# gstoica27/ReLUQP-py

Hardware: AMD Instinct MI355X
Metric: QP solves/sec (batch=4096 random dense QPs n=100 m=300) (higher is better)
Workload: dtype f32; 1 GPU; batch=4096/GPU random dense QPs n=100 m=300 (n_eq=25), feasible rand_qp seeds 0.., eps_abs=0.001, cold start, reference defaults; 4 distinct batches in rotation, every solve without dispatch history (= first solve of a fresh handle); global_batch=4096, parallelism=batch-split x1, no collectives, kernel=resident2, tile=same, low_memory=False, fresh_batches=4, dispatch_history=False, rho_window=5

## Files before the change

### reluqp-py_amd/csrc/rqp_resident2.hip

```cpp
#include <cstdio>
#include <cstdlib>
#include <type_traits>
#include <vector>

#include "rqp_common.h"

typedef float f2 __attribute__((ext_vector_type(2)));
typedef _Float16 h2 __attribute__((ext_vector_type(2)));

__device__ __forceinline__ float fma_mix_lo(h2 k, float v, float acc) {
    asm("v_fma_mix_f32 %0, %1, %2, %0 op_sel_hi:[1,0,0]" : "+v"(acc) : "v"(k), "v"(v));
    return acc;
}
__device__ __forceinline__ float fma_mix_hi(h2 k, float v, float acc) {
    asm("v_fma_mix_f32 %0, %1, %2, %0 op_sel:[1,0,0] op_sel_hi:[1,0,0]" : "+v"(acc) : "v"(k), "v"(v));
    return acc;
}
template <int CTRL>
__device__ __forceinline__ float dpp2(float v) {
    return __builtin_bit_cast(float, __builtin_amdgcn_update_dpp(0, __builtin_bit_cast(int, v), CTRL, 0xF, 0xF, true));
}
__device__ __forceinline__ float swsum32(float a, float b) {
    asm volatile("s_nop 1\n\tv_permlane32_swap_b32 %0, %1" : "+v"(a), "+v"(b));
    return a + b;
}
__device__ __forceinline__ float swsum16(float a, float b) {
    asm volatile("s_nop 1\n\tv_permlane16_swap_b32 %0, %1" : "+v"(a), "+v"(b));
    return a + b;
}
__device__ __forceinline__ float swmax32(float a, float b) {
    asm volatile("s_nop 1\n\tv_permlane32_swap_b32 %0, %1" : "+v"(a), "+v"(b));
    return fmaxf(a, b);
}
__device__ __forceinline__ float swmax16(float a, float b) {
    asm volatile("s_nop 1\n\tv_permlane16_swap_b32 %0, %1" : "+v"(a), "+v"(b));
    return fmaxf(a, b);
}
__device__ __forceinline__ float wave_max(float v) {
    v = fmaxf(v, dpp2<0xB1>(v));
    v = fmaxf(v, dpp2<0x4E>(v));
    v = fmaxf(v, dpp2<0x141>(v));
    v = fmaxf(v, dpp2<0x128>(v));
    float a = v, b = v;
    asm volatile("s_nop 1\n\tv_permlane16_swap_b32 %0, %1" : "+v"(a), "+v"(b));
    v = fmaxf(a, b);
    a = v; b = v;
    asm volatile("s_nop 1\n\tv_permlane32_swap_b32 %0, %1" : "+v"(a), "+v"(b));
    return fmaxf(a, b);
}
__device__ __forceinline__ unsigned wave_or(unsigned v) {
    v |= (unsigned)__builtin_amdgcn_update_dpp(0, (int)v, 0xB1, 0xF, 0xF, true);
    v |= (unsigned)__builtin_amdgcn_update_dpp(0, (int)v, 0x4E, 0xF, 0xF, true);
    v |= (unsigned)__builtin_amdgcn_update_dpp(0, (int)v, 0x141, 0xF, 0xF, true);
    v |= (unsigned)__builtin_amdgcn_update_dpp(0, (int)v, 0x128, 0xF, 0xF, true);
    unsigned a = v, b = v;
    asm volatile("s_nop 1\n\tv_permlane16_swap_b32 %0, %1" : "+v"(a), "+v"(b));
    v = a | b;
    a = v; b = v;
    asm volatile("s_nop 1\n\tv_permlane32_swap_b32 %0, %1" : "+v"(a), "+v"(b));
    return a | b;
}
template <typename T>
__device__ __forceinline__ T tmax2(T a, T b) {
    return (a != a) ? a : ((b != b) ? b : (a > b ? a : b));
}

template <int RB_, int CQ_, int KR_, int KC_>
struct Res2Cfg {
    static constexpr int RB = RB_, CQ = CQ_, KR = KR_, KC = KC_;
    static constexpr int NT = 256, NW = 4, NQ = 2, PL = 32;
    static constexpr int RP = RB / 2, KP = KR / 2;
    static constexpr int CW = NQ * CQ;
    static constexpr int N = NW * CW;
    static constexpr int M = PL * RB;
    static constexpr int SW = 8 * KR + 4;
    static constexpr int ND = NW * SW;
    static constexpr int AE2 = RP * CQ;
    static constexpr int KE2 = KP * KC;
    static constexpr int HR = 4, HP = HR / 2;
    static constexpr int HE2 = HP * CQ;
    static constexpr int HU = HE2 / 2;
    static constexpr int H1 = (CQ + 1) / 2, H2 = (H1 + 1) / 2;
    static constexpr int MATREGS = 2 * (RP * CQ + KP * KC);
    static constexpr int WAVES_PER_SIMD = (MATREGS > 100) ? 2 : ((MATREGS > 30) ? 3 : 4);
    static_assert(RB % 2 == 0 && KR % 2 == 0 && HP == 2 && HU == CQ && PL * HR >= N, "row pairs");
    static_assert(8 * KR >= CW && 8 * KC >= N && M <= 2 * NT && KC == CQ && NQ == 2, "tile shape");
    static constexpr size_t lds_bytes() {
        return (size_t)M * 8 * 4 + ND * 8 + 16 * 8
               + (size_t)M * 4 * 5
               + (size_t)ND * 4 * 6
               + (size_t)NW * M * 4 + 96 * 4
               + (size_t)HU * NT * 16;
    }
};

constexpr int NSEG = 25;
template <class C, bool DIAG, bool KH, bool KD = false>
__global__ void __launch_bounds__(256, C::WAVES_PER_SIMD) k_admm_res2(SolveArgs a, const float* __restrict__ Apack,
                                                      const float* __restrict__ Kpack,
                                                      const float* __restrict__ Hpack, unsigned long long* dbg,
                                                      const float* __restrict__ Kscale) {
    constexpr int RB = C::RB, CQ = C::CQ, KR = C::KR, KC = C::KC, NT = C::NT, NW = C::NW, RP = C::RP, KP = C::KP;
    constexpr int CW = C::CW, M = C::M, ND = C::ND, SW = C::SW, AE2 = C::AE2, KE2 = C::KE2, HU = C::HU, HP = C::HP, HR = C::HR, H1 = C::H1, H2 = C::H2;
    extern __shared__ __attribute__((aligned(16))) unsigned char smem_raw[];
    double* zt64 = (double*)smem_raw;
    double* lam64 = zt64 + M;
    double* z64 = lam64 + M;
    double* inv64 = z64 + M;
    double* x64 = inv64 + M;
    double* redd = x64 + ND;
    float* lT = (float*)(redd + 16);
    float* uT = lT + M;
    float* rv32 = uT + M;
    float* nu = rv32 + M;
    float* cT = nu + M;
    float* xin = cT + M;
    float* xnat = xin + ND;
    float* dxv = xnat + ND;
    float* hx = dxv + ND;
    float* gT = hx + ND;
    float* dvec = gT + ND;
    float* part = dvec + ND;
    float* red = part + NW * M;
    float* Hs = red + 96;
    static_assert(((size_t)M * 8 * 4 + ND * 8 + 16 * 8 + (size_t)M * 4 * 5 + ND * 4 * 6 + NW * M * 4 + 96 * 4) % 16 == 0,
                  "H image must start 16-byte aligned");

    const int n = a.n, m = a.m;
    const int b = a.order ? a.order[blockIdx.x] : (int)blockIdx.x, tid = threadIdx.x;
    const int wave = tid >> 6, lane = tid & 63;
    const int q = lane & 1, pl = lane >> 1, rr = lane >> 3, cc = lane & 7;
    const size_t mat = (a.sA == 0) ? 0 : (size_t)b;
    const float* cg = (const float*)a.c + (size_t)b * m;
    int k0 = 0;
    bool exact = false;
    if (a.cont == 1) {
        if (a.info.status[b] != RQP_STATUS_CONTINUE) {
            if (!(a.warm_starting || a.keep_state)) {
                for (int i = tid; i < n; i += NT) a.x[(size_t)b * n + i] = 0.0;
                for (int i = tid; i < m; i += NT) {
                    a.z[(size_t)b * m + i] = 0.0;
                    a.lam[(size_t)b * m + i] = 0.0;
                }
                if (tid == 0) a.rho_ind[b] = a.rho_ind0;
            }
            return;
        }
        k0 = a.cont_iter[b];
    } else if (a.cont == 2) {
        if (a.gate && *a.gate == 0) return;
        if (a.cstat[b] == 0) return;
        const int ci = a.cont_iter[b];
        if (ci >= 0) {
            k0 = ci;
            exact = true;
        }
    }
    const int wb = a.wbase ? a.wbase[mat] : 0;
    if (a.cstat && a.mode == 0) {
        const int sl = a.rho_ind[b] - wb;
        if (sl < 0 || sl >= a.kwin) {
            if (tid == 0) {
                a.cstat[b] = 1;
                if (!exact) a.cont_iter[b] = -1;
                atomicAdd(a.ncont, 1);
            }
            return;
        }
    }

    f2 ar[RP][CQ];
    {
        const f2* Ap = (const f2*)(Apack + mat * (size_t)AE2 * NT * 2) + tid;
#pragma unroll
        for (int rp = 0; rp < RP; ++rp)
#pragma unroll
            for (int c = 0; c < CQ; ++c) ar[rp][c] = Ap[(size_t)(rp * CQ + c) * NT];
        const float4* Hp = (const float4*)(Hpack + mat * (size_t)HU * NT * 4);
#pragma unroll
        for (int u = 0; u < HU; ++u) ((float4*)Hs)[u * NT + tid] = Hp[u * NT + tid];
    }
    int ri = a.rho_ind[b];
    float* rhoL = red + 64;
    if (tid < 32) rhoL[tid] = (tid < a.nrho) ? (float)a.rhos[tid] : 0.f;
    typedef typename std::conditional<KH, h2, f2>::type kpair_t;
    kpair_t kr[KP][KC];
    float kscale = 1.f;
    auto load_K = [&](int jl) {
        int j = jl - wb;
        j = j < 0 ? 0 : (j >= a.kwin ? a.kwin - 1 : j);
        if constexpr (!KD) {
            int tid_k = tid;
            asm volatile("" : "+v"(tid_k));
            const kpair_t* Kp = (const kpair_t*)Kpack + (mat * a.kwin + j) * (size_t)KE2 * NT + tid_k;
#pragma unroll
            for (int kp = 0; kp < KP; ++kp)
#pragma unroll
                for (int c = 0; c < KC; ++c) kr[kp][c] = Kp[(size_t)(kp * KC + c) * NT];
            if constexpr (KH) kscale = Kscale[mat * a.kwin + j];
        } else {
            int lane_o = lane, wave_o = wave;
            asm volatile("" : "+v"(lane_o), "+v"(wave_o));
            const int rr = lane_o >> 3, cc = lane_o & 7, wave = wave_o;
            const float* Kj = (const float*)a.K + ((a.sK == 0) ? (size_t)0 : (size_t)b * a.sK) + (size_t)j * n * a.ldn;
            typedef float f4u __attribute__((ext_vector_type(4), aligned(4)));
#pragma unroll
            for (int kp = 0; kp < KP; ++kp) {
                const int lr = KR * rr + 2 * kp, r = CW * wave + lr;
                const bool ok0 = lr < CW && r < n, ok1 = lr + 1 < CW && r + 1 < n;
                const float* row0 = Kj + (size_t)(r < n ? r : n - 1) * a.ldn + KC * cc;
                const float* row1 = Kj + (size_t)(r + 1 < n ? r + 1 : n - 1) * a.ldn + KC * cc;
                float t0[KC], t1[KC];
#pragma unroll
                for (int c = 0; c + 4 <= KC; c += 4) {
                    const f4u u0 = *(const f4u*)(row0 + c), u1 = *(const f4u*)(row1 + c);
#pragma unroll
                    for (int e = 0; e < 4; ++e) { t0[c + e] = u0[e]; t1[c + e] = u1[e]; }
                }
#pragma unroll
                for (int c = KC - KC % 4; c < KC; ++c) { t0[c] = row0[c]; t1[c] = row1[c]; }
                const f2 msk = {ok0 ? 1.f : 0.f, ok1 ? 1.f : 0.f};
#pragma unroll
                for (int c = 0; c < KC; ++c) kr[kp][c] = (f2){t0[c], t1[c]} * msk;
            }
        }
    };
    load_K(ri);

    auto set_rho_rows = [&](int j) {
        const float rho = (float)a.rhos[j];
        for (int i = tid; i < M; i += NT) {
            const float rv = rho * ((i < m) ? cg[i] : 1.f);
            rv32[i] = rv;
            inv64[i] = 1.0 / (double)rv;
        }
    };
    for (int i = tid; i < M; i += NT) {
        const bool in = i < m;
        zt64[i] = (exact && in) ? a.ax[(size_t)b * m + i] : 0.0;
        z64[i] = in ? a.z[(size_t)b * m + i] : 0.0;
        lam64[i] = in ? a.lam[(size_t)b * m + i] : 0.0;
        lT[i] = in ? ((const float*)a.l)[(size_t)b * m + i] : 0.f;
        uT[i] = in ? ((const float*)a.u)[(size_t)b * m + i] : 0.f;
        nu[i] = 0.f;
        cT[i] = in ? cg[i] : 1.f;
    }
    set_rho_rows(ri);
    for (int i = tid; i < ND; i += NT) {
        const int col = CW * (i / SW) + (i % SW);
        const bool in = (i % SW) < CW && col < n;
        const double xv = in ? a.x[(size_t)b * n + col] : 0.0;
        x64[i] = xv;
        xin[i] = (float)xv;
        xnat[i] = (i < n) ? (float)a.x[(size_t)b * n + i] : 0.f;
        gT[i] = in ? ((const float*)a.g)[(size_t)b * n + col] : 0.f;
        hx[i] = 0.f;
        dxv[i] = 0.f;
        dvec[i] = 0.f;
    }

    int colw, ncolw;
    {
        const int b5 = (lane >> 5) & 1, b4 = (lane >> 4) & 1;
        const int cbase = H2 * b4 + H1 * b5;
        int nval = b4 ? (H1 - H2) : H2;
        if (b5 && cbase + nval > CQ) nval = CQ - cbase;
        ncolw = ((lane & 0xE) == 0) ? nval : 0;
        colw = SW * wave + CQ * q + cbase;
    }
    __syncthreads();

    auto load_vc = [&](const float* v, float (&vc)[CQ]) __attribute__((always_inline)) {
#pragma unroll
        for (int c = 0; c < CQ; ++c) vc[c] = v[SW * wave + CQ * q + c];
    };
    auto prod_A = [&](const float (&vc)[CQ]) __attribute__((always_inline)) {
        f2 acc[RP];
#pragma unroll
        for (int rp = 0; rp < RP; ++rp) {
            f2 s = {0.f, 0.f};
#pragma unroll
            for (int c = 0; c < CQ; ++c) s = __builtin_elementwise_fma(ar[rp][c], (f2){vc[c], vc[c]}, s);
            s.x += dpp2<0xB1>(s.x);
            s.y += dpp2<0xB1>(s.y);
            acc[rp] = s;
        }
        if (q == 0) {
            f2* dst = (f2*)(part + wave * M + RB * pl);
#pragma unroll
            for (int rp = 0; rp < RP; ++rp) dst[rp] = acc[rp];
        }
    };
    auto prod_At = [&](auto use_a, auto use_h, const float* w, float* out, bool addg) {
        constexpr bool USE_A = decltype(use_a)::value, USE_H = decltype(use_h)::value;
        f2 wr[RP];
        f2 wx[HP];
        if constexpr (USE_A) {
#pragma unroll
            for (int rp = 0; rp < RP; ++rp) wr[rp] = ((const f2*)(w + RB * pl))[rp];
        }
        if constexpr (USE_H) {
            const float4 xv = *(const float4*)(xnat + HR * pl);
            wx[0] = (f2){xv.x, xv.y};
            wx[1] = (f2){xv.z, xv.w};
        }
        auto hload = [&](int c) -> float4 { return ((const float4*)Hs)[c * NT + tid]; };
        auto colsum = [&](int c, const float4& hv) -> float {
            f2 t2 = {0.f, 0.f};
            if constexpr (USE_A) {
#pragma unroll
                for (int rp = 0; rp < RP; ++rp) t2 = __builtin_elementwise_fma(ar[rp][c], wr[rp], t2);
            }
            if constexpr (USE_H) {
                t2 = __builtin_elementwise_fma((f2){hv.x, hv.y}, wx[0], t2);
                t2 = __builtin_elementwise_fma((f2){hv.z, hv.w}, wx[1], t2);
            }
            return t2.x + t2.y;
        };
        float s1[H1];
        auto colsum2 = [&](int c0, int c1, const float4& h0, const float4& h1, float& a0, float& a1) __attribute__((always_inline)) {
            f2 t0 = {0.f, 0.f}, t1 = {0.f, 0.f};
            if constexpr (USE_A) {
#pragma unroll
                for (int rp = 0; rp < RP; ++rp) {
                    t0 = __builtin_elementwise_fma(ar[rp][c0], wr[rp], t0);
                    t1 = __builtin_elementwise_fma(ar[rp][c1], wr[rp], t1);
                }
            }
            if constexpr (USE_H) {
                t0 = __builtin_elementwise_fma((f2){h0.x, h0.y}, wx[0], t0);
                t1 = __builtin_elementwise_fma((f2){h1.x, h1.y}, wx[0], t1);
                t0 = __builtin_elementwise_fma((f2){h0.z, h0.w}, wx[1], t0);
                t1 = __builtin_elementwise_fma((f2){h1.z, h1.w}, wx[1], t1);
            }
            a0 = t0.x + t0.y;
            a1 = t1.x + t1.y;
        };
        float4 hcur = {0.f, 0.f, 0.f, 0.f}, hnext = {0.f, 0.f, 0.f, 0.f};
        if constexpr (USE_H) {
            hcur = hload(0);
            if (H1 < CQ) hnext = hload(H1);
        }
#pragma unroll
        for (int i = 0; i < H1; ++i) {
            const bool pair = (i + H1 < CQ);
            if (pair) {
                float4 hc2 = hcur, hn2 = hnext;
                if constexpr (USE_H) {
                    if (i + 1 < H1) hc2 = hload(i + 1);
                    if (i + 1 + H1 < CQ) hn2 = hload(i + 1 + H1);
                }
                float a0, a1;
                colsum2(i, i + H1, hcur, hnext, a0, a1);
                s1[i] = swsum32(a0, a1);
                hcur = hc2;
                hnext = hn2;
            } else {
                const float a0 = colsum(i, hcur);
                s1[i] = swsum32(a0, a0);
            }
        }
        float gpre[H2];
#pragma unroll
        for (int i = 0; i < H2; ++i) gpre[i] = addg ? gT[colw + i] : 0.f;
        float s2[H2];
#pragma unroll
        for (int i = 0; i < H2; ++i) s2[i] = (i + H2 < H1) ? swsum16(s1[i], s1[i + H2]) : swsum16(s1[i], s1[i]);
#pragma unroll
        for (int i = 0; i < H2; ++i) {
            float v = s2[i];
            v += dpp2<0x4E>(v);
            v += dpp2<0x124>(v);
            v += dpp2<0x128>(v);
            s2[i] = v;
        }
        if (ncolw > 0) {
#pragma unroll
            for (int i = 0; i < H2; ++i)
                if (i < ncolw) out[colw + i] = s2[i] + gpre[i];
        }
    };
    constexpr std::true_type YES{};
    auto prod_At_chk = [&](const float* w, float* outA, float* outH) {
        f2 wr[RP];
        f2 wx[HP];
#pragma unroll
        for (int rp = 0; rp < RP; ++rp) wr[rp] = ((const f2*)(w + RB * pl))[rp];
        {
            const float4 xv = *(const float4*)(xnat + HR * pl);
            wx[0] = (f2){xv.x, xv.y};
            wx[1] = (f2){xv.z, xv.w};
        }
        auto hload = [&](int c) -> float4 { return ((const float4*)Hs)[c * NT + tid]; };
        float sA[H1], sH[H1];
        float4 hcur = hload(0), hnext = {0.f, 0.f, 0.f, 0.f};
        if (H1 < CQ) hnext = hload(H1);
#pragma unroll
        for (int i = 0; i < H1; ++i) {
            const bool pair = (i + H1 < CQ);
            float4 hc2 = hcur, hn2 = hnext;
            if (i + 1 < H1) hc2 = hload(i + 1);
            if (i + 1 + H1 < CQ) hn2 = hload(i + 1 + H1);
            f2 a0 = {0.f, 0.f}, a1 = {0.f, 0.f};
            f2 h0 = __builtin_elementwise_fma((f2){hcur.x, hcur.y}, wx[0], (f2){0.f, 0.f}), h1 = {0.f, 0.f};
            if (pair) h1 = __builtin_elementwise_fma((f2){hnext.x, hnext.y}, wx[0], h1);
#pragma unroll
            for (int rp = 0; rp < RP; ++rp) {
                a0 = __builtin_elementwise_fma(ar[rp][i], wr[rp], a0);
                if (pair) a1 = __builtin_elementwise_fma(ar[rp][i + H1], wr[rp], a1);
            }
            h0 = __builtin_elementwise_fma((f2){hcur.z, hcur.w}, wx[1], h0);
            if (pair) h1 = __builtin_elementwise_fma((f2){hnext.z, hnext.w}, wx[1], h1);
            const float ca0 = a0.x + a0.y, ch0 = h0.x + h0.y;
            sA[i] = pair ? swsum32(ca0, a1.x + a1.y) : swsum32(ca0, ca0);
            sH[i] = pair ? swsum32(ch0, h1.x + h1.y) : swsum32(ch0, ch0);
            hcur = hc2;
            hnext = hn2;
        }
        float tA[H2], tH[H2];
#pragma unroll
        for (int i = 0; i < H2; ++i) {
            tA[i] = (i + H2 < H1) ? swsum16(sA[i], sA[i + H2]) : swsum16(sA[i], sA[i]);
            tH[i] = (i + H2 < H1) ? swsum16(sH[i], sH[i + H2]) : swsum16(sH[i], sH[i]);
        }
#pragma unroll
        for (int i = 0; i < H2; ++i) {
            float va = tA[i], vh = tH[i];
            va += dpp2<0x4E>(va);
            vh += dpp2<0x4E>(vh);
            va += dpp2<0x124>(va);
            vh += dpp2<0x124>(vh);
            va += dpp2<0x128>(va);
            vh += dpp2<0x128>(vh);
            tA[i] = va;
            tH[i] = vh;
        }
        if (ncolw > 0) {
#pragma unroll
            for (int i = 0; i < H2; ++i)
                if (i < ncolw) {
                    outA[colw + i] = tA[i] + 0.f;
                    outH[colw + i] = tH[i] + 0.f;
                }
        }
    };
    auto prod_K = [&](const float* v, float (&s)[KR]) {
        float vc[KC];
#pragma unroll
        for (int c = 0; c < KC; ++c) vc[c] = v[SW * (cc >> 1) + CQ * (cc & 1) + c];
#pragma unroll
        for (int kp = 0; kp < KP; ++kp) {
            f2 t = {0.f, 0.f};
            if constexpr (KH) {
#pragma unroll
                for (int c = 0; c < KC; ++c) {
                    t.x = fma_mix_lo(kr[kp][c], vc[c], t.x);
                    t.y = fma_mix_hi(kr[kp][c], vc[c], t.y);
                }
                t.x *= kscale;
                t.y *= kscale;
            } else {
#pragma unroll
                for (int c = 0; c < KC; ++c) t = __builtin_elementwise_fma(kr[kp][c], (f2){vc[c], vc[c]}, t);
            }
            s[2 * kp] = t.x;
            s[2 * kp + 1] = t.y;
        }
#pragma unroll
        for (int r = 0; r < KR; ++r) s[r] += dpp2<0xB1>(s[r]);
#pragma unroll
        for (int r = 0; r < KR; ++r) s[r] += dpp2<0x4E>(s[r]);
#pragma unroll
        for (int r = 0; r < KR; ++r) s[r] += dpp2<0x141>(s[r]);
    };
    float cv[3] = {0.f, 0.f, 0.f};
    auto row_body = [&](auto nr, bool init, bool do_a, bool do_b, bool chk) __attribute__((always_inline)) {
        constexpr int R = decltype(nr)::value;
        double zt[R], z[R], lmv[R], iv[R];
        float adx[R][NW], lo[R], hi[R], rvf[R];
#pragma unroll
        for (int q = 0; q < R; ++q) {
            const int i = tid + q * NT;
            zt[q] = zt64[i];
            lmv[q] = lam64[i];
            if (do_a) {
                iv[q] = inv64[i];
                lo[q] = lT[i];
                hi[q] = uT[i];
            } else {
                z[q] = z64[i];
            }
            rvf[q] = rv32[i];
            if (init || do_a) {
#pragma unroll
                for (int w = 0; w < NW; ++w) adx[q][w] = part[w * M + i];
            }
        }
        asm volatile("s_waitcnt lgkmcnt(0)" ::: "memory");
#pragma unroll
        for (int q = 0; q < R; ++q) {
            asm volatile("" : "+v"(zt[q]), "+v"(lmv[q]), "+v"(rvf[q]));
            if (do_a) asm volatile("" : "+v"(iv[q]), "+v"(lo[q]), "+v"(hi[q]));
            else asm volatile("" : "+v"(z[q]));
            if (init || do_a) asm volatile("" : "+v"(adx[q][0]), "+v"(adx[q][1]), "+v"(adx[q][2]), "+v"(adx[q][3]));
        }
#pragma unroll
        for (int q = 0; q < R; ++q) {
            const int i = tid + q * NT;
            if (init || do_a) {
                const float ad = ((adx[q][0] + adx[q][1]) + adx[q][2]) + adx[q][3];
                zt[q] = (init ? 0.0 : zt[q]) + (double)ad;
                zt64[i] = zt[q];
            }
            if (do_a) {
                const double v = zt[q] + lmv[q] * iv[q];
                z[q] = v;
                if (v < (double)lo[q]) z[q] = (double)lo[q];
                if (v > (double)hi[q]) z[q] = (double)hi[q];
                z64[i] = z[q];
            }
            if (do_b) {
                const double rv = (double)rvf[q];
                const double pr = zt[q] - z[q];
                const double lh = lmv[q] + rv * pr;
                lam64[i] = lh;
                nu[i] = (float)(lh + rv * pr);
            }
        }
        if (chk) {
            int tid_w = tid;
            asm volatile("" : "+v"(tid_w));
#pragma unroll
            for (int q = 0; q < R; ++q) {
                const int i = tid_w + q * NT;
                const float we = (a.scE && i < m) ? (float)(1.0 / a.scE[mat * m + i]) : 1.f;
                nu[i] = (float)lmv[q];
                cv[0] = tmax2(cv[0], fabsf((float)(zt[q] - z[q])) * we);
                cv[1] = tmax2(cv[1], fabsf((float)zt[q]) * we);
                cv[2] = tmax2(cv[2], fabsf((float)z[q]) * we);
            }
        }
    };
    auto row_pass = [&](bool init, bool do_a, bool do_b, bool chk = false) __attribute__((always_inline)) {
        if constexpr (M > NT) {
            static_assert(M <= 2 * NT, "at most two rows per lane");
            if (tid + NT < M) {
                row_body(std::integral_constant<int, 2>{}, init, do_a, do_b, chk);
                return;
            }
        }
        if (tid < M) row_body(std::integral_constant<int, 1>{}, init, do_a, do_b, chk);
    };

    __builtin_amdgcn_s_waitcnt(0x0F70);
    unsigned long long t_last = 0, t_acc[NSEG] = {};
    bool k_pend = false;
    bool diag_on = true;
    auto stamp = [&](int seg) {
        if constexpr (DIAG) {
            __builtin_amdgcn_sched_barrier(0);
            unsigned long long t;
            asm volatile("s_memtime %0\n\ts_waitcnt lgkmcnt(0)" : "=s"(t)::"memory");
            __builtin_amdgcn_sched_barrier(0);
            if (seg >= 0 && diag_on) t_acc[seg] += t - t_last;
            t_last = t;
        }
    };

    float rho_est = (a.mode == 2) ? (float)a.rho_in : ((a.cont == 1 || exact) ? (float)a.cont_rho[b] : (float)a.rhos[ri]);
    float pri = 0.f, dua = 0.f;
    bool converged = false;
    int iters = k0;
    const float tolT = (float)a.tol;
    const int kmax = (a.mode == 2) ? 0 : a.max_iter;

    if (!exact) {
        float vc0[CQ];
        load_vc(xin, vc0);
        prod_A(vc0);
        __syncthreads();
        row_pass(true, false, kmax > k0);
    } else {
        row_pass(false, false, kmax > k0);
    }

    float scl_p = 0.f, scl_d = 0.f;
    auto res_rows = [&]() {
        cv[0] = cv[1] = cv[2] = 0.f;
        int tid_w = tid;
        asm volatile("" : "+v"(tid_w));
        for (int i = tid_w; i < M; i += NT) {
            const float we = (a.scE && i < m) ? (float)(1.0 / a.scE[mat * m + i]) : 1.f;
            nu[i] = (float)lam64[i];
            cv[0] = tmax2(cv[0], fabsf((float)(zt64[i] - z64[i])) * we);
            cv[1] = tmax2(cv[1], fabsf((float)zt64[i]) * we);
            cv[2] = tmax2(cv[2], fabsf((float)z64[i]) * we);
        }
    };
    int rpar = 0;
    auto residuals = [&](float rho_carry, float& o_pri, float& o_dua) -> float {
        float v[7];
#pragma unroll
        for (int e = 0; e < 3; ++e) v[e] = cv[e];
#pragma unroll
        for (int e = 3; e < 7; ++e) v[e] = 0.f;
        int tid_w = tid;
        asm volatile("" : "+v"(tid_w));
        __syncthreads();
        stamp(10);
        if (tid < ND && (tid % SW) >= CW) {
            dxv[tid] = 0.f;
            hx[tid] = 0.f;
        }
        prod_At_chk(nu, dxv, hx);
        stamp(11);
        __syncthreads();
        stamp(13);
        if (tid < ND) {
            float wd = 1.f;
            if (a.scD) {
                const int col = CW * (tid_w / SW) + (tid_w % SW);
                if ((tid_w % SW) < CW && col < n) wd = (float)(1.0 / (a.scC[mat] * a.scD[mat * n + col]));
            }
            const float t3 = dxv[tid];
            v[3] = fabsf(hx[tid] + t3 + gT[tid]) * wd;
            v[4] = fabsf(hx[tid]) * wd;
            v[5] = fabsf(t3) * wd;
            v[6] = fabsf(gT[tid]) * wd;
        }
        unsigned nanm = 0;
#pragma unroll
        for (int e = 0; e < 7; ++e) nanm |= (__builtin_amdgcn_ballot_w64(v[e] != v[e]) != 0ull) ? (1u << e) : 0u;
        float u0, u1;
        {
            const float r0 = swmax32(v[0], v[4]), r1 = swmax32(v[1], v[5]), r2 = swmax32(v[2], v[6]), r3 = swmax32(v[3], v[3]);
            u0 = swmax16(r0, r2);
            u1 = swmax16(r1, r3);
        }
        u0 = fmaxf(u0, dpp2<0xB1>(u0));
        u1 = fmaxf(u1, dpp2<0xB1>(u1));
        u0 = fmaxf(u0, dpp2<0x4E>(u0));
        u1 = fmaxf(u1, dpp2<0x4E>(u1));
        u0 = fmaxf(u0, dpp2<0x141>(u0));
        u1 = fmaxf(u1, dpp2<0x141>(u1));
        u0 = fmaxf(u0, dpp2<0x128>(u0));
        u1 = fmaxf(u1, dpp2<0x128>(u1));
        float* redp = red + 32 * rpar;
        rpar ^= 1;
        if ((lane & 15) == 0) {
            const int row = lane >> 4;
            *(f2*)(redp + wave * 8 + 2 * row) = (f2){u0, row == 3 ? __builtin_bit_cast(float, nanm) : u1};
        }
        stamp(14);
        __syncthreads();
        stamp(15);
        nanm = 0;
#pragma unroll
        for (int w = 0; w < NW; ++w) nanm |= __builtin_bit_cast(unsigned, redp[w * 8 + 7]);
#pragma unroll
        for (int e = 0; e < 7; ++e) {
            float r = redp[e];
#pragma unroll
            for (int w = 1; w < NW; ++w) r = fmaxf(r, redp[w * 8 + e]);
            v[e] = ((nanm >> e) & 1u) ? __builtin_nanf("") : r;
        }
        stamp(16);
        o_pri = v[0];
        o_dua = v[3];
        scl_p = tmax2(v[1], v[2]);
        scl_d = tmax2(tmax2(v[4], v[5]), v[6]);
        const float num = v[0] / scl_p;
        const float den = v[3] / scl_d;
        float est = rho_carry * sqrtf(num / den);
        if (est < (float)a.rho_min) est = (float)a.rho_min;
        if (est > (float)a.rho_max) est = (float)a.rho_max;
        return est;
    };

    stamp(-1);
    int to_chk = a.check_interval - (k0 % a.check_interval);
    for (int k = k0 + 1; k <= kmax; ++k) {
        __syncthreads();
        stamp(0);
        prod_At(YES, YES, nu, dvec, true);
        stamp(1);
        __syncthreads();
        stamp(2);
        __builtin_amdgcn_s_waitcnt(0x0F70);
        if constexpr (DIAG) {
            if (k_pend) { stamp(20); k_pend = false; }
        }
        {
            float s[KR];
            static_assert(KR == 4 || KR == 2, "vectorised x update");
            const int j = SW * wave + KR * rr;
            double2* xp = (double2*)(x64 + j);
            double2 xold[KR / 2];
#pragma unroll
            for (int hlf = 0; hlf < KR / 2; ++hlf) xold[hlf] = xp[hlf];
            prod_K(dvec, s);
            if (cc == 0) {
#pragma unroll
                for (int hlf = 0; hlf < KR / 2; ++hlf) ((f2*)(dxv + j))[hlf] = (f2){-s[2 * hlf], -s[2 * hlf + 1]};
            }
            __builtin_amdgcn_fence(__ATOMIC_RELEASE, "wavefront");
            __builtin_amdgcn_wave_barrier();
            float vc[CQ];
            load_vc(dxv, vc);
            if (cc == 0) {
                f2* xn2 = (f2*)(xnat + CW * wave + KR * rr);
#pragma unroll
                for (int hlf = 0; hlf < KR / 2; ++hlf) {
                    double2 xa = xold[hlf];
                    const f2 dx = {-s[2 * hlf], -s[2 * hlf + 1]};
                    xa.x += (double)dx.x;
                    xa.y += (double)dx.y;
                    xp[hlf] = xa;
                    const f2 xf = {(float)xa.x, (float)xa.y};
                    ((f2*)(xin + j))[hlf] = xf;
                    if (KR * rr + 2 * hlf + 1 < CW) xn2[hlf] = xf;
                }
            }
            stamp(3);
            prod_A(vc);
        }
        stamp(4);
        __syncthreads();
        stamp(5);
        stamp(6);
        iters = k;
        const bool on_grid = (--to_chk == 0);
        if (on_grid) to_chk = a.check_interval;
        const bool check = (a.mode == 0) && on_grid;
        if (!check) {
            row_pass(false, true, k < kmax);
            stamp(7);
        } else {
            cv[0] = cv[1] = cv[2] = 0.f;
            row_pass(false, true, false, true);
            stamp(8);
            if constexpr (DIAG) t_acc[22] += 1;
            const int ri_before = ri;
            rho_est = residuals(rho_est, pri, dua);
            rho_est = __builtin_bit_cast(float, __builtin_amdgcn_readfirstlane(__builtin_bit_cast(int, rho_est)));
            pri = __builtin_bit_cast(float, __builtin_amdgcn_readfirstlane(__builtin_bit_cast(int, pri)));
            dua = __builtin_bit_cast(float, __builtin_amdgcn_readfirstlane(__builtin_bit_cast(int, dua)));
            if (rho_est > rhoL[ri] * tolT && ri < a.nrho - 1)
                ri += 1;
            else if (rho_est < rhoL[ri] / tolT && ri > 0)
                ri -= 1;
            if (a.info.trace && (k / a.check_interval) <= a.info.trace_cap && tid == 0) {
                double* tr = a.info.trace + ((size_t)b * a.info.trace_cap + (k / a.check_interval - 1)) * 4;
                tr[0] = (double)pri; tr[1] = (double)dua; tr[2] = (double)rho_est; tr[3] = (double)ri_before;
            }
            float tp = (float)a.thr_p, td = (float)a.thr_d;
            if (a.eps_rel > 0) {
                tp += (float)a.eps_rel * __builtin_bit_cast(float, __builtin_amdgcn_readfirstlane(__builtin_bit_cast(int, scl_p)));
                td += (float)a.eps_rel * __builtin_bit_cast(float, __builtin_amdgcn_readfirstlane(__builtin_bit_cast(int, scl_d)));
            }
            stamp(18);
            if (pri < tp && dua < td) {
                converged = true;
                break;
            }
            if (ri != ri_before) {
                if (a.cstat && k < kmax && (ri < wb || ri >= wb + a.kwin)) {
                    int tid_o = tid;
                    asm volatile("" : "+v"(tid_o));
                    for (int i = tid_o; i < n; i += NT) a.x[(size_t)b * n + i] = x64[SW * (i / CW) + i % CW];
                    for (int i = tid_o; i < m; i += NT) {
                        a.z[(size_t)b * m + i] = z64[i];
                        a.lam[(size_t)b * m + i] = lam64[i];
                        a.ax[(size_t)b * m + i] = zt64[i];
                    }
                    if (tid_o == 0) {
                        a.rho_ind[b] = ri;
                        a.cont_iter[b] = k;
                        a.cont_rho[b] = (double)rho_est;
                        a.cstat[b] = 1;
                        atomicAdd(a.ncont, 1);
                    }
                    return;
                }
                if constexpr (DIAG) { t_acc[23] += 1; k_pend = true; }
                if constexpr (!KD) load_K(ri);
                {
                    int tid_o = tid;
                    asm volatile("" : "+v"(tid_o));
                    const float rho = rhoL[ri];
                    for (int i = tid_o; i < M; i += NT) {
                        const float rv = rho * cT[i];
                        rv32[i] = rv;
                        inv64[i] = 1.0 / (double)rv;
                    }
                }
                if constexpr (KD) load_K(ri);
                stamp(19);
            }
            if (k < kmax) row_pass(false, false, true);
            stamp(21);
        }
    }
    if constexpr (DIAG) {
        diag_on = false;
        if (lane == 0)
            for (int e = 0; e < NSEG; ++e) dbg[((size_t)b * 4 + wave) * NSEG + e] = (e == NSEG - 1) ? (unsigned long long)iters : t_acc[e];
    }

    __syncthreads();
    if (a.mode == 1) {
        for (int i = tid; i < n; i += NT) a.x[(size_t)b * n + i] = x64[SW * (i / CW) + i % CW];
        for (int i = tid; i < m; i += NT) {
            a.z[(size_t)b * m + i] = z64[i];
            a.lam[(size_t)b * m + i] = lam64[i];
        }
        return;
    }
    if (!converged) {
        res_rows();
        rho_est = residuals(rho_est, pri, dua);
    }

    double jp = 0.0;
    if (tid < ND) jp = (double)(xin[tid] * (0.5f * hx[tid] + gT[tid]));
    for (int off = 32; off >= 1; off >>= 1) jp += __shfl_xor(jp, off, 64);
    if (lane == 0) redd[wave] = jp;
    __syncthreads();
    const double obj = redd[0] + redd[1] + redd[2] + redd[3];

    if (a.mode == 2) {
        if (tid == 0) {
            if (a.r_pri) a.r_pri[b] = (double)pri;
            if (a.r_dua) a.r_dua[b] = (double)dua;
            if (a.r_rho) a.r_rho[b] = (double)rho_est;
            if (a.r_obj) a.r_obj[b] = obj;
        }
        return;
    }

    if (a.out_x) for (int i = tid; i < n; i += NT) ((float*)a.out_x)[(size_t)b * n + i] = (float)x64[SW * (i / CW) + i % CW];
    if (a.out_z) for (int i = tid; i < m; i += NT) ((float*)a.out_z)[(size_t)b * m + i] = (float)z64[i];
    if (a.out_lam) for (int i = tid; i < m; i += NT) ((float*)a.out_lam)[(size_t)b * m + i] = (float)lam64[i];
    if (tid == 0) {
        if (a.cstat) a.cstat[b] = 0;
        if (a.info.iter) a.info.iter[b] = converged ? iters : a.max_iter;
        if (a.last_iter) a.last_iter[b] = converged ? iters : a.max_iter;
        if (a.info.status) a.info.status[b] = converged ? RQP_STATUS_SOLVED : ((pri != pri || dua != dua) ? RQP_STATUS_NAN : RQP_STATUS_MAX_ITER);
        if (a.info.rho_ind) a.info.rho_ind[b] = ri;
        if (a.info.pri_res) a.info.pri_res[b] = (double)pri;
        if (a.info.dua_res) a.info.dua_res[b] = (double)dua;
        if (a.info.rho_estimate) a.info.rho_estimate[b] = (double)rho_est;
        if (a.info.obj_val) a.info.obj_val[b] = obj;
    }
    if ((a.warm_starting || a.keep_state)) {
        for (int i = tid; i < n; i += NT) a.x[(size_t)b * n + i] = x64[SW * (i / CW) + i % CW];
        for (int i = tid; i < m; i += NT) {
            a.z[(size_t)b * m + i] = z64[i];
            a.lam[(size_t)b * m + i] = lam64[i];
        }
        if (tid == 0) a.rho_ind[b] = ri;
    } else {
        for (int i = tid; i < n; i += NT) a.x[(size_t)b * n + i] = 0.0;
        for (int i = tid; i < m; i += NT) {
            a.z[(size_t)b * m + i] = 0.0;
            a.lam[(size_t)b * m + i] = 0.0;
        }
        if (tid == 0) a.rho_ind[b] = a.rho_ind0;
    }
}

template <class C, bool KH>
__global__ void k_pack_res2(int n, int ldn, int nrho, const float* __restrict__ K, float* __restrict__ Kpack, float* __restrict__ Kscale,
                            const int32_t* __restrict__ only, const int32_t* __restrict__ gate) {
    constexpr int KR = C::KR, KC = C::KC, NT = C::NT, CW = C::CW, KE2 = C::KE2;
    const int mat = blockIdx.y;
    if (gate && *gate == 0) return;
    if (only && !only[mat]) return;
    const int t = threadIdx.x, w = t >> 6, lane = t & 63;
    const int rr = lane >> 3, cc = lane & 7;
    extern __shared__ __attribute__((aligned(16))) float stage[];
    {
        const int j = blockIdx.x;
        const float* Kj = K + ((size_t)mat * nrho + j) * n * ldn;
        for (int i = t; i < n * ldn; i += NT) stage[i] = Kj[i];
        __syncthreads();
        float inv_scale = 1.f;
        if constexpr (KH) {
            __shared__ float smax[NT];
            float mx = 0.f;
            for (int i = t; i < n * ldn; i += NT) mx = fmaxf(mx, fabsf(stage[i]));
            smax[t] = mx;
            __syncthreads();
            for (int off = NT / 2; off >= 1; off >>= 1) {
                if (t < off) smax[t] = fmaxf(smax[t], smax[t + off]);
                __syncthreads();
            }
            int e2 = 0;
            (void)frexpf(fmaxf(smax[0], 1e-30f), &e2);
            const float sc = ldexpf(1.f, e2 - 14);
            inv_scale = ldexpf(1.f, 14 - e2);
            if (t == 0) Kscale[(size_t)mat * nrho + j] = sc;
        }
        float* Kp = Kpack + ((size_t)mat * nrho + j) * KE2 * NT * (KH ? 1 : 2);
        for (int pair = 0; pair < KE2; ++pair) {
            const int lr = KR * rr + 2 * (pair / KC);
            const int r = CW * w + lr, c = KC * cc + pair % KC;
            f2 v;
            v.x = (lr < CW && r < n && c < n) ? stage[r * ldn + c] : 0.f;
            v.y = (lr + 1 < CW && r + 1 < n && c < n) ? stage[(r + 1) * ldn + c] : 0.f;
            if constexpr (KH)
                ((h2*)Kp)[(size_t)pair * NT + t] = (h2){(_Float16)(v.x * inv_scale), (_Float16)(v.y * inv_scale)};
            else
                ((f2*)Kp)[(size_t)pair * NT + t] = v;
        }
    }
}


template <class C>
__global__ void k_pack_res2_ah(int n, int m, int ldn, const float* __restrict__ A, const float* __restrict__ Ht,
                               float* __restrict__ Apack, float* __restrict__ Hpack) {
    constexpr int RB = C::RB, CQ = C::CQ, NT = C::NT, CW = C::CW, AE2 = C::AE2, HU = C::HU, HR = C::HR, RCH = C::M / 4;
    const int mat = blockIdx.y, ch = blockIdx.x, t = threadIdx.x;
    extern __shared__ __attribute__((aligned(16))) float stage[];
    if (ch < 4) {
        if (!A) return;
        const int r0 = RCH * ch;
        const float* Am = A + (size_t)mat * m * ldn + (size_t)r0 * ldn;
        const int avail = (m - r0) * ldn;
        if ((((size_t)Am) & 15) == 0) {
            for (int i = 4 * t; i < RCH * ldn; i += 4 * NT)
                *(float4*)(stage + i) = (i < avail) ? *(const float4*)(Am + i) : (float4){0.f, 0.f, 0.f, 0.f};
        } else {
            for (int i = t; i < RCH * ldn; i += NT) stage[i] = (i < avail) ? Am[i] : 0.f;
        }
        __syncthreads();
        const int l16 = t & 15, w = (t >> 4) & 3, part = t >> 6;
        const int lane = 16 * ch + l16, q = lane & 1, pl = lane >> 1, tk = 64 * w + lane;
        f2* Ap = (f2*)(Apack + (size_t)mat * AE2 * NT * 2);
        for (int pair = part; pair < AE2; pair += 4) {
            const int lr = RB * pl + 2 * (pair / CQ) - r0, c = CW * w + CQ * q + pair % CQ;
            f2 v;
            v.x = (c < n) ? stage[lr * ldn + c] : 0.f;
            v.y = (c < n) ? stage[(lr + 1) * ldn + c] : 0.f;
            Ap[(size_t)pair * NT + tk] = v;
        }
    } else {
        const int w = t >> 6, lane = t & 63, q = lane & 1, pl = lane >> 1;
        const float* Hm = Ht + (size_t)mat * n * ldn;
        if ((((size_t)Hm) & 15) == 0) {
            for (int i = 4 * t; i < n * ldn; i += 4 * NT) *(float4*)(stage + i) = *(const float4*)(Hm + i);
        } else {
            for (int i = t; i < n * ldn; i += NT) stage[i] = Hm[i];
        }
        __syncthreads();
        float4* Hp = (float4*)(Hpack + (size_t)mat * HU * NT * 4);
        for (int c0 = 0; c0 < CQ; ++c0) {
            const int c = CW * w + CQ * q + c0;
            float hv[HR];
            for (int h = 0; h < HR; ++h) {
                const int r = HR * pl + h;
                hv[h] = (r < n && c < n) ? stage[c * ldn + r] : 0.f;
            }
            Hp[(size_t)c0 * NT + t] = (float4){hv[0], hv[1], hv[2], hv[3]};
        }
    }
}

typedef Res2Cfg<10, 13, 4, 13> Cfg2C2;
typedef Res2Cfg<2, 4, 2, 4> Cfg2C4;
typedef Res2Cfg<4, 7, 2, 7> Cfg2M;
typedef Res2Cfg<10, 10, 4, 10> Cfg2N;

static int res2_pick(const rqp_handle* h) {
    if (h->esz != 4 || h->nrho > 32) return -1;
    if (h->n <= Cfg2C4::N && h->m <= Cfg2C4::M) return 0;
    if (h->n <= Cfg2M::N && h->m <= Cfg2M::M) return 1;
    if (h->n <= Cfg2N::N && h->m <= Cfg2N::M) return 3;
    if (h->n <= Cfg2C2::N && h->m <= Cfg2C2::M) return 2;
    return -1;
}

bool rqp_res2_fits(const rqp_handle* h) { return res2_pick(h) >= 0; }

template <class C>
static void pack_elems_t(const rqp_handle* h, size_t* a_elems, size_t* k_elems, size_t* h_elems) {
    *a_elems = (size_t)h->nmat * C::AE2 * C::NT * 2;
    *k_elems = h->k_direct ? 0 : (size_t)h->nmat * h->kwin * C::KE2 * C::NT * (h->dims.tile_dtype == RQP_TILE_F16 ? 1 : 2);
    *h_elems = (size_t)h->nmat * C::HU * C::NT * 4;
}
void rqp_res2_pack_elems(const rqp_handle* h, size_t* a_elems, size_t* k_elems, size_t* h_elems) {
    switch (res2_pick(h)) {
        case 0: pack_elems_t<Cfg2C4>(h, a_elems, k_elems, h_elems); break;
        case 1: pack_elems_t<Cfg2M>(h, a_elems, k_elems, h_elems); break;
        case 3: pack_elems_t<Cfg2N>(h, a_elems, k_elems, h_elems); break;
        default: pack_elems_t<Cfg2C2>(h, a_elems, k_elems, h_elems); break;
    }
}

void rqp_res2_kp_layout(const rqp_handle* h, int* cw, int* kr, int* kc) {
    switch (res2_pick(h)) {
        case 0: *cw = Cfg2C4::CW; *kr = Cfg2C4::KR; *kc = Cfg2C4::KC; break;
        case 1: *cw = Cfg2M::CW; *kr = Cfg2M::KR; *kc = Cfg2M::KC; break;
        case 3: *cw = Cfg2N::CW; *kr = Cfg2N::KR; *kc = Cfg2N::KC; break;
        default: *cw = Cfg2C2::CW; *kr = Cfg2C2::KR; *kc = Cfg2C2::KC; break;
    }
}

template <class C>
static hipError_t pack_t(const rqp_handle* h, const void* A_src, const int32_t* only, const int32_t* gate, hipStream_t s) {
    const size_t stage_ah = (size_t)(C::M / 4 > h->n ? C::M / 4 : h->n) * h->ldn * sizeof(float);
    const size_t stage_k = (size_t)h->n * h->ldn * sizeof(float);
    if (!only)
        k_pack_res2_ah<C><<<dim3(5, h->nmat), C::NT, stage_ah, s>>>(h->n, h->m, h->ldn, (const float*)A_src, (const float*)h->Ht, h->Apack, h->Hpack);
    if (h->dims.tile_dtype == RQP_TILE_F16) {
        k_pack_res2<C, true><<<dim3(h->kwin, h->nmat), C::NT, stage_k, s>>>(h->n, h->ldn, h->kwin, (const float*)h->K, h->Kpack, h->Kscale, only, gate);
    } else {
        if (!h->k_direct && !h->kpack_direct)
            k_pack_res2<C, false><<<dim3(h->kwin, h->nmat), C::NT, stage_k, s>>>(h->n, h->ldn, h->kwin, (const float*)h->K, h->Kpack, nullptr, only, gate);
    }
    return hipGetLastError();
}
hipError_t rqp_launch_pack_res2(const rqp_handle* h, const void* A_src, const int32_t* only, const int32_t* gate, hipStream_t s) {
    switch (res2_pick(h)) {
        case 0: return pack_t<Cfg2C4>(h, A_src, only, gate, s);
        case 1: return pack_t<Cfg2M>(h, A_src, only, gate, s);
        case 3: return pack_t<Cfg2N>(h, A_src, only, gate, s);
        default: return pack_t<Cfg2C2>(h, A_src, only, gate, s);
    }
}

template <class C>
static hipError_t prepare_t(const rqp_handle* h) {
    const size_t lds = C::lds_bytes();
    {
        const size_t stage_ah = (size_t)(C::M / 4 > h->n ? C::M / 4 : h->n) * h->ldn * sizeof(float);
        hipError_t ae = rqp_raise_lds_limit((const void*)k_pack_res2_ah<C>, stage_ah);
        if (ae != hipSuccess) return ae;
    }
    {
        const size_t stage = (size_t)h->n * h->ldn * sizeof(float);
        hipError_t pe = (h->dims.tile_dtype == RQP_TILE_F16)
                            ? rqp_raise_lds_limit((const void*)k_pack_res2<C, true>, (size_t)stage)
                            : rqp_raise_lds_limit((const void*)k_pack_res2<C, false>, (size_t)stage);
        if (pe != hipSuccess) return pe;
    }
    if (h->dims.tile_dtype == RQP_TILE_F16)
        return rqp_raise_lds_limit((const void*)k_admm_res2<C, false, true>, (size_t)lds);
    hipError_t e = rqp_raise_lds_limit((const void*)k_admm_res2<C, false, false>, (size_t)lds);
    if (e != hipSuccess) return e;
    if (h->k_direct) {
        e = rqp_raise_lds_limit((const void*)k_admm_res2<C, false, false, true>, (size_t)lds);
        if (e != hipSuccess) return e;
    }
    if (h->debug & 2) e = rqp_raise_lds_limit((const void*)k_admm_res2<C, true, false>, (size_t)lds);
    if (h->debug & 1) {
        int nb = -1;
        hipError_t oe = hipOccupancyMaxActiveBlocksPerMultiprocessor(&nb, k_admm_res2<C, false, false>, C::NT, lds);
        hipFuncAttributes fa;
        (void)hipFuncGetAttributes(&fa, (const void*)k_admm_res2<C, false, false>);
        fprintf(stderr, "[rqp] k_admm_res2<%d,%d,%d,%d>: blocks/CU=%d (err %d) lds=%zu B regs=%d scratch=%zu B\n", C::RB, C::CQ,
                C::KR, C::KC, nb, (int)oe, lds, fa.numRegs, (size_t)fa.localSizeBytes);
    }
    return e;
}
hipError_t rqp_prepare_res2(const rqp_handle* h) {
    switch (res2_pick(h)) {
        case 0: return prepare_t<Cfg2C4>(h);
        case 1: return prepare_t<Cfg2M>(h);
        case 3: return prepare_t<Cfg2N>(h);
        default: return prepare_t<Cfg2C2>(h);
    }
}

template <class C>
static hipError_t solve_t(const rqp_handle* h, const SolveArgs& a, hipStream_t s) {
    const size_t lds = C::lds_bytes();
    if (h->dims.tile_dtype == RQP_TILE_F16) {
        k_admm_res2<C, false, true><<<h->B, C::NT, lds, s>>>(a, h->Apack, h->Kpack, h->Hpack, nullptr, h->Kscale);
        return hipGetLastError();
    }
    if ((h->debug & 2) && !h->k_direct) {
        const std::vector<double> sums = rqp_diag_run(s, h->B, 4, NSEG, [&](unsigned long long* dbg) {
            k_admm_res2<C, true, false><<<h->B, C::NT, lds, s>>>(a, h->Apack, h->Kpack, h->Hpack, dbg, nullptr);
        });
        if (sums.empty()) return hipErrorOutOfMemory;
        static const char* names[22] = {"B3 wait", "A'nu+Hx", "B1 wait", "Kd+x", "A dx", "B2 wait", "-", "rows",
                                        "rows(a)", "res rows", "R1 wait", "A'lam", "Hx", "R2 wait", "norms+reduce", "R3 wait", "combine",
                                        "R4 wait", "decision", "K issue+rho rows", "K wait", "rows(b)"};
        for (int w = 0; w < 4; ++w) {
            const double* tot = &sums[(size_t)w * NSEG];
            const double its = tot[NSEG - 1], chk = tot[22] > 0 ? tot[22] : 1.0;
            fprintf(stderr, "[rqp diag] wave %d cycles/iteration:", w);
            double sum = 0, csum = 0;
            for (int e = 8; e < 22; ++e) csum += tot[e];
            for (int e = 0; e < 8; ++e) { fprintf(stderr, " %s=%.0f", names[e], tot[e] / its); sum += tot[e] / its; }
            fprintf(stderr, " check=%.0f | total=%.0f\n", csum / its, sum + csum / its);
            fprintf(stderr, "[rqp diag] wave %d cycles/check:", w);
            for (int e = 8; e < 22; ++e) fprintf(stderr, " %s=%.0f", names[e], tot[e] / chk);
            fprintf(stderr, " | total=%.0f ; checks/instance=%.2f moves/instance=%.2f moves/check=%.3f\n", csum / chk, tot[22] / h->B,
                    tot[23] / h->B, tot[23] / chk);
        }
        return hipGetLastError();
    }
    if (h->k_direct)
        k_admm_res2<C, false, false, true><<<h->B, C::NT, lds, s>>>(a, h->Apack, nullptr, h->Hpack, nullptr, nullptr);
    else
        k_admm_res2<C, false, false><<<h->B, C::NT, lds, s>>>(a, h->Apack, h->Kpack, h->Hpack, nullptr, nullptr);
    return hipGetLastError();
}
hipError_t rqp_launch_solve_res2(const rqp_handle* h, const SolveArgs& a, hipStream_t s) {
    switch (res2_pick(h)) {
        case 0: return solve_t<Cfg2C4>(h, a, s);
        case 1: return solve_t<Cfg2M>(h, a, s);
        case 3: return solve_t<Cfg2N>(h, a, s);
        default: return solve_t<Cfg2C2>(h, a, s);
    }
}
```

Baseline: 1.408 million QP/s.

## Rearrange LDS layout and spread the x update across lanes

```diff
diff --git a/reluqp-py_amd/csrc/rqp_resident2.hip b/reluqp-py_amd/csrc/rqp_resident2.hip
--- a/reluqp-py_amd/csrc/rqp_resident2.hip
+++ b/reluqp-py_amd/csrc/rqp_resident2.hip
@@ -75,6 +75,9 @@
     static constexpr int M = PL * RB;
     static constexpr int SW = 8 * KR + 4;
     static constexpr int ND = NW * SW;
+    static constexpr bool TRI = 2 * ND + CQ - 1 > 255;
+    static constexpr int TW = TRI ? 3 * SW : SW;
+    static constexpr int TA = TRI ? SW : ND;
     static constexpr int AE2 = RP * CQ;
     static constexpr int KE2 = KP * KC;
     static constexpr int HR = 4, HP = HR / 2;
@@ -86,9 +89,10 @@
     static_assert(RB % 2 == 0 && KR % 2 == 0 && HP == 2 && HU == CQ && PL * HR >= N, "row pairs");
     static_assert(8 * KR >= CW && 8 * KC >= N && M <= 2 * NT && KC == CQ && NQ == 2, "tile shape");
     static constexpr size_t lds_bytes() {
-        return (size_t)M * 8 * 4 + ND * 8 + 16 * 8
-               + (size_t)M * 4 * 5
-               + (size_t)ND * 4 * 6
+        return (size_t)ND * 4 * 3 + (size_t)M * 4 + ND * 4
+               + (size_t)M * 8 * 4 + ND * 8 + 16 * 8
+               + (size_t)M * 4 * 4
+               + (size_t)ND * 4 * 2
                + (size_t)NW * M * 4 + 96 * 4
                + (size_t)HU * NT * 16;
     }
@@ -101,9 +105,14 @@
                                                       const float* __restrict__ Hpack, unsigned long long* dbg,
                                                       const float* __restrict__ Kscale) {
     constexpr int RB = C::RB, CQ = C::CQ, KR = C::KR, KC = C::KC, NT = C::NT, NW = C::NW, RP = C::RP, KP = C::KP;
-    constexpr int CW = C::CW, M = C::M, ND = C::ND, SW = C::SW, AE2 = C::AE2, KE2 = C::KE2, HU = C::HU, HP = C::HP, HR = C::HR, H1 = C::H1, H2 = C::H2;
+    constexpr int CW = C::CW, M = C::M, ND = C::ND, SW = C::SW, TW = C::TW, TA = C::TA, AE2 = C::AE2, KE2 = C::KE2, HU = C::HU, HP = C::HP, HR = C::HR, H1 = C::H1, H2 = C::H2;
     extern __shared__ __attribute__((aligned(16))) unsigned char smem_raw[];
-    double* zt64 = (double*)smem_raw;
+    float* dvec = (float*)smem_raw;
+    float* dxv = dvec + TA;
+    float* gT = dxv + TA;
+    float* nu = dvec + 3 * ND;
+    float* xin = nu + M;
+    double* zt64 = (double*)(xin + ND);
     double* lam64 = zt64 + M;
     double* z64 = lam64 + M;
     double* inv64 = z64 + M;
@@ -112,20 +121,24 @@
     float* lT = (float*)(redd + 16);
     float* uT = lT + M;
     float* rv32 = uT + M;
-    float* nu = rv32 + M;
-    float* cT = nu + M;
-    float* xin = cT + M;
-    float* xnat = xin + ND;
-    float* dxv = xnat + ND;
-    float* hx = dxv + ND;
-    float* gT = hx + ND;
-    float* dvec = gT + ND;
-    float* part = dvec + ND;
+    float* cT = rv32 + M;
+    float* xnat = cT + M;
+    float* hx = dvec;
+    float* part = xnat + 2 * ND;
+    static_assert(2 * ND >= C::PL * HR, "xnat covers the H rows of every lane group");
     float* red = part + NW * M;
     float* Hs = red + 96;
-    static_assert(((size_t)M * 8 * 4 + ND * 8 + 16 * 8 + (size_t)M * 4 * 5 + ND * 4 * 6 + NW * M * 4 + 96 * 4) % 16 == 0,
-                  "H image must start 16-byte aligned");
-
+    static_assert(((size_t)ND * 4 * 4 + M * 4) % 16 == 0 && ((size_t)M * 8 * 4 + ND * 8 + 16 * 8 + (size_t)M * 4 * 4) % 16 == 0 &&
+                      ((size_t)ND * 4 * 2 + NW * M * 4 + 96 * 4) % 16 == 0,
+                  "the doubles, xnat and the H image must start 16-byte aligned");
+    static_assert(3 * ND * 4 + (RP - 1) * 8 <= 255 * 8 && 2 * TA + CQ - 1 <= 255, "nu / gT within reach of the ds_read2 offsets");
+    auto tslot = [](int i) { return C::TRI ? i + (TW - SW) * (i / SW) : i; };
+    auto tslot_o = [&]() {
+        if constexpr (!C::TRI) return (int)threadIdx.x;
+        int t = threadIdx.x;
+        asm volatile("" : "+v"(t));
+        return t + (TW - SW) * (t / SW);
+    };
     const int n = a.n, m = a.m;
     const int b = a.order ? a.order[blockIdx.x] : (int)blockIdx.x, tid = threadIdx.x;
     const int wave = tid >> 6, lane = tid & 63;
@@ -253,10 +266,10 @@
         x64[i] = xv;
         xin[i] = (float)xv;
         xnat[i] = (i < n) ? (float)a.x[(size_t)b * n + i] : 0.f;
-        gT[i] = in ? ((const float*)a.g)[(size_t)b * n + col] : 0.f;
-        hx[i] = 0.f;
-        dxv[i] = 0.f;
-        dvec[i] = 0.f;
+        xnat[ND + i] = 0.f;
+        gT[tslot(i)] = in ? ((const float*)a.g)[(size_t)b * n + col] : 0.f;
+        dxv[tslot(i)] = 0.f;
+        dvec[tslot(i)] = 0.f;
     }
 
     int colw, ncolw;
@@ -266,13 +279,13 @@
         int nval = b4 ? (H1 - H2) : H2;
         if (b5 && cbase + nval > CQ) nval = CQ - cbase;
         ncolw = ((lane & 0xE) == 0) ? nval : 0;
-        colw = SW * wave + CQ * q + cbase;
+        colw = TW * wave + CQ * q + cbase;
     }
     __syncthreads();
 
-    auto load_vc = [&](const float* v, float (&vc)[CQ]) __attribute__((always_inline)) {
-#pragma unroll
-        for (int c = 0; c < CQ; ++c) vc[c] = v[SW * wave + CQ * q + c];
+    auto load_vc = [&](const float* v, int pitch, float (&vc)[CQ]) __attribute__((always_inline)) {
+#pragma unroll
+        for (int c = 0; c < CQ; ++c) vc[c] = v[pitch * wave + CQ * q + c];
     };
     auto prod_A = [&](const float (&vc)[CQ]) __attribute__((always_inline)) {
         f2 acc[RP];
@@ -447,7 +460,7 @@
     auto prod_K = [&](const float* v, float (&s)[KR]) {
         float vc[KC];
 #pragma unroll
-        for (int c = 0; c < KC; ++c) vc[c] = v[SW * (cc >> 1) + CQ * (cc & 1) + c];
+        for (int c = 0; c < KC; ++c) vc[c] = v[TW * (cc >> 1) + CQ * (cc & 1) + c];
 #pragma unroll
         for (int kp = 0; kp < KP; ++kp) {
             f2 t = {0.f, 0.f};
@@ -576,7 +589,7 @@
 
     if (!exact) {
         float vc0[CQ];
-        load_vc(xin, vc0);
+        load_vc(xin, SW, vc0);
         prod_A(vc0);
         __syncthreads();
         row_pass(true, false, kmax > k0);
@@ -609,8 +622,8 @@
         __syncthreads();
         stamp(10);
         if (tid < ND && (tid % SW) >= CW) {
-            dxv[tid] = 0.f;
-            hx[tid] = 0.f;
+            dxv[tslot_o()] = 0.f;
+            hx[tslot_o()] = 0.f;
         }
         prod_At_chk(nu, dxv, hx);
         stamp(11);
@@ -622,11 +635,12 @@
                 const int col = CW * (tid_w / SW) + (tid_w % SW);
                 if ((tid_w % SW) < CW && col < n) wd = (float)(1.0 / (a.scC[mat] * a.scD[mat * n + col]));
             }
-            const float t3 = dxv[tid];
-            v[3] = fabsf(hx[tid] + t3 + gT[tid]) * wd;
-            v[4] = fabsf(hx[tid]) * wd;
+            const int ts = tslot_o();
+            const float t3 = dxv[ts], t2 = hx[ts];
+            v[3] = fabsf(t2 + t3 + gT[ts]) * wd;
+            v[4] = fabsf(t2) * wd;
             v[5] = fabsf(t3) * wd;
-            v[6] = fabsf(gT[tid]) * wd;
+            v[6] = fabsf(gT[ts]) * wd;
         }
         unsigned nanm = 0;
 #pragma unroll
@@ -693,33 +707,23 @@
         {
             float s[KR];
             static_assert(KR == 4 || KR == 2, "vectorised x update");
-            const int j = SW * wave + KR * rr;
-            double2* xp = (double2*)(x64 + j);
-            double2 xold[KR / 2];
-#pragma unroll
-            for (int hlf = 0; hlf < KR / 2; ++hlf) xold[hlf] = xp[hlf];
+            const int jr = KR * rr + cc;
+            double* xp = x64 + SW * wave + jr;
+            double xa = 0.0;
+            if (cc < KR) xa = *xp;
             prod_K(dvec, s);
-            if (cc == 0) {
-#pragma unroll
-                for (int hlf = 0; hlf < KR / 2; ++hlf) ((f2*)(dxv + j))[hlf] = (f2){-s[2 * hlf], -s[2 * hlf + 1]};
-            }
+            float sr = s[0];
+#pragma unroll
+            for (int r = 1; r < KR; ++r) sr = (cc == r) ? s[r] : sr;
+            if (cc < KR) dxv[TW * wave + jr] = -sr;
             __builtin_amdgcn_fence(__ATOMIC_RELEASE, "wavefront");
             __builtin_amdgcn_wave_barrier();
             float vc[CQ];
-            load_vc(dxv, vc);
-            if (cc == 0) {
-                f2* xn2 = (f2*)(xnat + CW * wave + KR * rr);
-#pragma unroll
-                for (int hlf = 0; hlf < KR / 2; ++hlf) {
-                    double2 xa = xold[hlf];
-                    const f2 dx = {-s[2 * hlf], -s[2 * hlf + 1]};
-                    xa.x += (double)dx.x;
-                    xa.y += (double)dx.y;
-                    xp[hlf] = xa;
-                    const f2 xf = {(float)xa.x, (float)xa.y};
-                    ((f2*)(xin + j))[hlf] = xf;
-                    if (KR * rr + 2 * hlf + 1 < CW) xn2[hlf] = xf;
-                }
+            load_vc(dxv, TW, vc);
+            if (cc < KR) {
+                xa += (double)(-sr);
+                *xp = xa;
+                if (jr < CW) xnat[CW * wave + jr] = (float)xa;
             }
             stamp(3);
             prod_A(vc);
@@ -822,7 +826,7 @@
     }
 
     double jp = 0.0;
-    if (tid < ND) jp = (double)(xin[tid] * (0.5f * hx[tid] + gT[tid]));
+    if (tid < ND) jp = (double)((float)x64[tid] * (0.5f * hx[tslot_o()] + gT[tslot_o()]));
     for (int off = 32; off >= 1; off >>= 1) jp += __shfl_xor(jp, off, 64);
     if (lane == 0) redd[wave] = jp;
     __syncthreads();
```

Result: faster. 1.520 million QP/s, median of 6 (+8.0%).
